# AI-ON/Few-Shot-Music-Generation

Measured on AMD Instinct MI355X. Metric: episodes/s (LSTM-baseline train step, synthetic vocab=10k seq_len=128 5-way/5-shot h=512), higher is better.
Workload: dtype f32 (bf16x3-split products, fp32 accumulate)

## Files before the change

### few-shot-music-generation_amd/csrc/api_forward.hip

```cpp
#include "fsmg_model.h"

using namespace fsmg;
using namespace fsmg_host;

namespace fsmg_host {

int stage_tokens(fsmg_model* h, const int32_t* support, int n_sup, const int32_t* query, int n_qry, int on_device) {
    const size_t T = h->T;
    if (on_device && h->eager_call) {
        h->cur_sup = support; h->cur_qry = query;
        return FSMG_OK;
    }
    const hipMemcpyKind kind = on_device ? hipMemcpyDeviceToDevice : hipMemcpyHostToDevice;
    if (n_sup > 0) HIPCK(h, hipMemcpyAsync(h->d_tok, support, sizeof(int) * n_sup * T, kind, h->stream));
    if (n_qry > 0) HIPCK(h, hipMemcpyAsync(h->d_tok + n_sup * T, query, sizeof(int) * n_qry * T, kind, h->stream));
    h->cur_sup = h->d_tok; h->cur_qry = h->d_tok + n_sup * T;
    return FSMG_OK;
}

int reset_tok_table(fsmg_model* h) {
    if (!h->tok_first) return FSMG_OK;
    OpBatch ops(h);
    GEMMCK(ops.add(h->tok_first, 0x7FFFFFFFu, h->V1));
    GEMMCK(ops.add(h->tok_count, 0u, h->V1));
    return ops.flush();
}

int token_prep(fsmg_model* h, int n_sup, int n_qry, bool train) {
    const bool table = train && h->tok_first != nullptr;
    HIPCK(h, launch_token_prep(h->stream, h->cur_sup, n_sup, h->cur_qry, n_qry, h->T, h->V, h->V,
                               h->X, h->Y, h->d_err, table ? h->tok_first : nullptr, table ? h->tok_count : nullptr));
    return FSMG_OK;
}

GemmArgs logits_args(fsmg_model* h, int B, int t0, int t1) {
    const int Hp = h->Hp;
    const int64_t r0 = (int64_t)t0 * B, m = (int64_t)(t1 - t0) * B;
    GemmArgs g{};
    g.A = h->Hs[h->L - 1] + (size_t)B * Hp + (size_t)r0 * Hp; g.lda = Hp;
    g.B = h->P + h->off_w; g.ldb = h->V1p;
    g.C = h->logits + (size_t)r0 * h->V1p; g.ldc = h->V1p; g.M = (int)m; g.N = h->V1p; g.K = Hp;
    g.bias = h->P + h->off_d; g.ksplit = 1; g.nt_store = 1;
    return g;
}
inline void fused_softmax_args(fsmg_model* h, GemmArgs& g) {
    g.ce_part = h->ce_part; g.ce_nvocab = h->V1; g.ce_store = 1;
}
int ce_finish(fsmg_model* h, hipStream_t s, int B, int64_t rows) {
    ScopedTimer tm(h, "ce");
    HIPCK(h, launch_ce_finish(s, h->ce_part, h->ce_nparts, h->Y, (int)rows, (float)(1.0 / ((double)rows + 1e-12)), h->logits, h->V1p,
                              h->lse, h->ce, h->crow, h->Hs[h->L - 1] + (size_t)B * h->Hp, h->Hsc, h->Hp, h->d_err, h->d_counters + 4));
    return FSMG_OK;
}
int ce_rows(fsmg_model* h, hipStream_t s, int B, int t0, int t1, int64_t rows_total) {
    ScopedTimer tm(h, "ce");
    const int64_t r0 = (int64_t)t0 * B, m = (int64_t)(t1 - t0) * B;
    HIPCK(h, launch_ce_rows(s, h->logits + (size_t)r0 * h->V1p, h->V1p, (int)m, h->V1, h->Y + r0, h->lse + r0,
                            h->ce + r0, dlogits_buf(h) + (size_t)r0 * h->V1p, (float)(1.0 / ((double)rows_total + 1e-12))));
    return FSMG_OK;
}

int logits_and_ce(fsmg_model* h, const Lane& ln, int B, int t0, int t1, int64_t rows_total, bool want_dlogits) {
    const int64_t r0 = (int64_t)t0 * B, m = (int64_t)(t1 - t0) * B;
    GemmArgs g = logits_args(h, B, t0, t1);
    if (!want_dlogits) {
        ScopedTimer tm(h, "gemm_logits");
        g.ce_part = h->ce_part + (size_t)r0 * h->ce_nparts; g.ce_tgt = h->Y + r0; g.ce_tgt_logit = h->tgt_logit + r0;
        g.ce_nvocab = h->V1; g.bx3 = h->bx3;
        if (use_h_gemm(h, OP_KC, OP_XC, g, ln)) g.bx3 = 3;
        else if (use_ws_gemm(h, OP_KC, OP_XC, g, ln)) { g.bx3 = 2; g.group_m = 4; }
        HIPCK(h, launch_gemm(ln.s, OP_KC, OP_XC, g, ln.lds_pad));
        HIPCK(h, launch_ce_combine(ln.s, h->ce_part + (size_t)r0 * h->ce_nparts, h->ce_nparts,
                                   h->tgt_logit + r0, (int)m, h->ce + r0));
        return FSMG_OK;
    }
// ... 219 lines not shown
```

### few-shot-music-generation_amd/csrc/api_handle.hip

```cpp
#include <mutex>
#include "fsmg_model.h"

using namespace fsmg;
using namespace fsmg_host;

namespace fsmg_host {

thread_local std::string g_create_error;

static int pick_concurrent_aux(fsmg_model* h, int priority, int max_tries) {
    if (max_tries <= 0) {
        if (hipStreamCreateWithPriority(&h->aux, hipStreamNonBlocking, priority) != hipSuccess) return fail(h, FSMG_ERR_HIP, "aux stream create failed");
        h->aux_tries = 0;
        return FSMG_OK;
    }
    int* d = nullptr;
    if (hipMalloc((void**)&d, 256) != hipSuccess) return fail(h, FSMG_ERR_NOMEM, "hipMalloc(queue probe) failed");
    auto probe = [&](hipStream_t cand, long long ticks) -> int {
        int seen = 0;
        const int init[2] = {0, -1};
        if (hipStreamSynchronize(h->stream) != hipSuccess || hipMemcpy(d, init, sizeof(init), hipMemcpyHostToDevice) != hipSuccess ||
            launch_queue_probe(h->stream, d, d + 1, 0, ticks) != hipSuccess || launch_queue_probe(cand, d, d + 1, 1, 0) != hipSuccess ||
            hipStreamSynchronize(cand) != hipSuccess || hipStreamSynchronize(h->stream) != hipSuccess ||
            hipMemcpy(&seen, d + 1, sizeof(int), hipMemcpyDeviceToHost) != hipSuccess) return -1;
// ... 100 lines not shown
        return fail(nullptr, FSMG_ERR_NO_DEVICE, std::string("libfsmg is built for gfx950 only, device is ") + prop.gcnArchName);

    fsmg_model* h = new (std::nothrow) fsmg_model();
    if (!h) return fail(nullptr, FSMG_ERR_NOMEM, "host allocation failed");
    h->cfg = *cfg;
    h->device = cfg->device;
    compute_dims(*cfg, h);
    h->n_flat = build_layout(h);
    auto bail = [&](int code, const std::string& msg) { g_create_error = msg; fsmg_destroy(h); return code; };

    if (cfg->stream) { h->stream = (hipStream_t)cfg->stream; h->own_stream = false; }
    else {
        if (hipStreamCreateWithFlags(&h->stream, hipStreamNonBlocking) != hipSuccess) return bail(FSMG_ERR_HIP, "hipStreamCreate failed");
        h->own_stream = true;
    }
    {
        if (const char* eg = std::getenv("FSMG_GRAPH")) h->cfg.use_graph = (eg[0] != '0');
        h->overlap = (int64_t)h->V1 >= 8LL * h->H * h->L;
        if (cfg->schedule == FSMG_SCHEDULE_SINGLE_STREAM) { h->overlap = false; h->overlap_forced = true; }
        if (cfg->schedule == FSMG_SCHEDULE_TWO_STREAM) { h->overlap = true; h->overlap_forced = true; }
        if (cfg->schedule == FSMG_SCHEDULE_XCD_PARTITIONED) h->xov = true;
        if (cfg->gemm == FSMG_GEMM_F32) h->bx3 = 0;
        if (cfg->recurrence == FSMG_RECURRENCE_PER_STEP) h->persist = false;
        if (cfg->recurrence == FSMG_RECURRENCE_COLUMN_SPLIT) h->xcd = false;
        if (cfg->recurrence == FSMG_RECURRENCE_XCD_LOCAL) h->pair_mode = 2;
        if (cfg->dp_split_backward) h->dp_split = cfg->dp_split_backward == 2 ? 2 : 1;
        const char* env = std::getenv("FSMG_OVERLAP");
        if (env) { h->overlap = env[0] != '0'; h->overlap_forced = true; }
        if (const char* e = std::getenv("FSMG_GEMM")) h->bx3 = std::strcmp(e, "f32") != 0;
        if (const char* e = std::getenv("FSMG_XCD_OVERLAP")) h->xov = std::atoi(e) != 0;
        if (const char* e = std::getenv("FSMG_XOV_PARTS")) h->xov_parts = std::max(1, std::min(7, std::atoi(e)));
        if (const char* e = std::getenv("FSMG_EAGER")) h->eager = (e[0] != '0');
        if (const char* e = std::getenv("FSMG_MERGE_DK")) h->merge_dk = (e[0] != '0');
        if (const char* e = std::getenv("FSMG_UPD_SPLIT")) h->upd_split = (e[0] != '0');
        if (const char* e = std::getenv("FSMG_TAIL_ASIDE")) h->tail_aside = (e[0] != '0');
        if (const char* e = std::getenv("FSMG_LAZY_CS")) h->lazy_cs = (e[0] != '0');
        if (const char* e = std::getenv("FSMG_FUSED_SOFTMAX")) h->fused_softmax = (e[0] != '0');

        if (const char* e = std::getenv("FSMG_INPLACE_DLOGITS")) h->inplace_dlogits = (e[0] != '0');
        if (const char* e = std::getenv("FSMG_XOV_SELFCHECK")) h->xov_selfcheck_left = std::max(0, std::atoi(e));
        if (const char* e = std::getenv("FSMG_XOV_SELFCHECK_EVERY")) h->xov_selfcheck_every = std::max(0, std::atoi(e));
        if (const char* e = std::getenv("FSMG_PERSISTENT")) h->persist = (e[0] != '0');
        h->persist_cfg = h->persist;
        if (const char* e = std::getenv("FSMG_FALLBACK_STEPS")) h->fallback_steps = std::max(1, std::atoi(e));
        if (const char* e = std::getenv("FSMG_XCD")) h->xcd = (e[0] != '0');
        if (const char* e = std::getenv("FSMG_XCD_PAIR")) h->pair_mode = std::max(0, std::min(2, std::atoi(e)));
        if (const char* e = std::getenv("FSMG_FWD_RT")) h->force_fwd_rt = (e[0] != '0');
        if (const char* e = std::getenv("FSMG_CHAIN_SPIN_LIMIT")) h->chain_spin_limit = std::max(0, std::atoi(e));
        if (const char* e = std::getenv("FSMG_XCD_VARIANT")) h->xcd_variant = std::atoi(e);
        if (const char* e = std::getenv("FSMG_XCD_VARIANT_BWD")) h->xcd_variant_bwd = std::atoi(e);
#ifdef FSMG_EXPERIMENTS
        if (const char* e = std::getenv("FSMG_CE_TAIL")) h->ce_tail = (e[0] != '0');
        if (const char* e = std::getenv("FSMG_CE_TAIL_BLOCKS")) h->ce_tail_blocks = std::max(1, std::min(4096, std::atoi(e)));
        if (const char* e = std::getenv("FSMG_XOV_DW_SPLIT")) h->xov_dw_split = std::max(1, std::atoi(e));
        if (const char* e = std::getenv("FSMG_XOV_PUB")) h->xov_pub = std::max(1, std::min(64, std::atoi(e)));
        if (const char* e = std::getenv("FSMG_FILL_EARLY")) h->fill_early = (e[0] != '0');
        if (const char* e = std::getenv("FSMG_FILLS_LATE")) h->fills_late = (e[0] != '0');
        if (const char* e = std::getenv("FSMG_XOV_TAIL")) h->xov_tail = std::max(0, std::min(64, std::atoi(e)));
        if (const char* e = std::getenv("FSMG_BWD_RS")) h->bwd_rs = (e[0] != '0');
        if (const char* e = std::getenv("FSMG_DP_SPLIT")) h->dp_split = std::max(0, std::min(2, std::atoi(e)));
        if (const char* e = std::getenv("FSMG_XCD_MAX_ROWS")) h->xcd_max_rows = std::max(1, std::min(128, std::atoi(e)));
        if (const char* e = std::getenv("FSMG_PERSIST_FWD")) h->persist_fwd = (e[0] != '0');
        if (const char* e = std::getenv("FSMG_PERSIST_BWD")) h->persist_bwd = (e[0] != '0');
        if (const char* e = std::getenv("FSMG_NCHUNK")) h->nchunk = h->nchunk_persist = std::max(1, std::min((int)fsmg_model::NCHUNK, std::atoi(e)));
        if (const char* e = std::getenv("FSMG_CHUNK_STEPS")) {
            std::vector<int> edges{0};
// ... 276 lines not shown
```

### few-shot-music-generation_amd/csrc/api_schedule.hip

```cpp
#include "fsmg_model.h"

using namespace fsmg;
using namespace fsmg_host;

namespace fsmg_host {

bool use_ws_gemm(fsmg_model* h, int amode, int bmode, const GemmArgs& g, const Lane& ln) {
    static const int mode = std::getenv("FSMG_GEMM_WS") ? std::atoi(std::getenv("FSMG_GEMM_WS")) : 1;
    if (!h->bx3 || mode == 0 || ln.lds_pad != 0 || g.xcd_first != 0) return false;
    if (mode == 2) return true;
    const int64_t tiles = ((g.M + 127) / 128) * (int64_t)((g.N + 127) / 128);
    if (amode == OP_KC && bmode == OP_XC) return g.K >= 384 && g.K <= 640 && tiles >= 512;
    if (amode == OP_XC && bmode == OP_XC) return tiles >= 256 && g.M <= 512;
    return g.K <= 4096;
}

bool use_h_gemm(fsmg_model* h, int amode, int bmode, const GemmArgs& g, const Lane& ln) {
    static const int mode = std::getenv("FSMG_GEMM_H") ? std::atoi(std::getenv("FSMG_GEMM_H")) : 1;
    if (!h->bx3 || mode == 0 || ln.lds_pad != 0 || g.xcd_first != 0) return false;
    if (amode == OP_XC && g.gather != nullptr && g.m_split == 0) return false;
    if (mode == 2) return true;
    const int64_t tiles = ((g.M + 255) / 256) * (int64_t)((g.N + 255) / 256);
    if (amode == OP_KC && bmode == OP_KC) return g.K >= 4096 && tiles >= 32;
    if (amode == OP_XC && bmode == OP_XC) {
        if (g.m_split > 0 && tiles >= 64) return g.K >= 896;
        return g.K >= 2048 && tiles >= 16;
    }
    return g.K >= 384 && tiles >= 512;
}

int gemm(fsmg_model* h, const Lane& ln, int amode, int bmode, GemmArgs g, OpBatch* defer, double* sq, bool* sq_done) {
    hipStream_t s = ln.s;
    g.bx3 = h->bx3;
    if (sq_done) *sq_done = false;
    int slots = ln.slots, tile_mn = 0;
    if (use_h_gemm(h, amode, bmode, g, ln)) {
        g.bx3 = 3; slots = 256; tile_mn = 256;
    } else if (use_ws_gemm(h, amode, bmode, g, ln)) {
        g.bx3 = 2; slots = 512 * 4 / 3;
        if (amode == OP_KC && bmode == OP_XC) g.group_m = 4;
    }
    const int S = (g.ldc == g.N) ? pick_split(g.M, g.N, g.K, slots, g.bx3 != 0, tile_mn) : 1;
    const int64_t mn = (int64_t)g.M * g.N;
    float* slabs = ln.slabs; float* cslabs = ln.colsum_slabs;
    bool deferred = false;
    if (S > 1 && defer != nullptr && ln.s == h->stream && h->arena != nullptr) {
        const int64_t need = round_up((int64_t)S * mn, 64) + (g.colsum ? round_up((int64_t)S * g.N, 64) : 0);
        if (h->arena_off + need <= h->arena_cap) {
            slabs = h->arena + h->arena_off; cslabs = slabs + round_up((int64_t)S * mn, 64);
            h->arena_off += need;
            deferred = true;
        }
    }
    if (S <= 1 || (!deferred && (int64_t)S * mn > h->slab_cap)) {
        if (S > 1 && !h->warned_split) {
            h->warned_split = true;
            fprintf(stderr, "[fsmg] split-K of a %d x %d x %d GEMM dropped: %d slabs do not fit the slab buffer (%lld floats)\n", g.M, g.N, g.K, S, (long long)h->slab_cap);
        }
        g.ksplit = 1;
        HIPCK(h, launch_gemm(s, amode, bmode, g, ln.lds_pad));
        if (g.row_scale != nullptr) HIPCK(h, launch_scale_rows(s, g.C, g.row_scale, g.M, g.N));
        return FSMG_OK;
    }
    if (!deferred && slabs == h->slabs && h->slabs_owner != nullptr) GEMMCK(h->slabs_owner->flush());
    if (!deferred && slabs == h->slabs && h->side_pending) {
        HIPCK(h, hipStreamWaitEvent(h->stream, h->ev_side, 0));
// ... 14 lines not shown
    }
    HIPCK(h, launch_reduce_slabs2(s, slabs, mn, S, C, mn, cslabs, g.N, colsum, colsum ? g.N : 0));
    if (g.row_scale != nullptr) HIPCK(h, launch_scale_rows(s, C, g.row_scale, g.M, g.N));
    return FSMG_OK;
}

int select_xcd_format(fsmg_model* h, int B) {
    if (h->Hp != 1024 || !h->bx3 || h->xcd_bx3_forced || h->khx == nullptr || !(h->persist && h->xcd)) return FSMG_OK;
    const bool want = lstm_xcd_bx3_pays(B, (int)h->Hp) && B <= h->xcd_max_rows;
    if (want == h->xcd_bx3) return FSMG_OK;
    h->xcd_bx3 = want;
    drop_graphs(h);
    return repack_recurrent_weights(h, h->stream);
}

void choose_schedule(fsmg_model* h, int B, bool train) {
    h->ov_call = h->overlap && (h->overlap_forced || !use_xcd(h, B));
    h->xov_call = false;
    h->eager_call = h->eager && !h->ov_call && h->persist && h->persist_fwd && h->persist_bwd &&
                    (use_xcd(h, B) || lstm_fwd_chain_supported(B, h->Hp) || lstm_fwd_chain_rt_supported(B, h->Hp));
    if (train && h->xov && ((h->Hp == 512 && h->L == 1) || h->Hp == 1024) && h->xcd_bx3 && h->bx3 && !h->ov_call && h->aux != nullptr && use_xcd(h, B) && h->persist_fwd && h->persist_bwd &&
        (!h->timing || h->timing_only == "lstm_fwd" || h->timing_only == "lstm_bwd")) {
        const int rpx = lstm_xcd16_packed_rows(B, h->Hp);
        h->xov_call = rpx > 0 && xov_first_free(B, h->Hp) <= (h->Hp == 1024 ? 6 : 5);
        if (h->xov_call) h->eager_call = true;
    }
}
void xov_gate(fsmg_model* h, GemmArgs& g, int B) {
    const int rpx = lstm_xcd16_packed_rows(B, h->Hp);
    g.gate = h->xov_prog; g.gate_expect = lstm_xcd_active_blocks(B, rpx, h->Hp); g.gate_rows = B; g.gate_last = h->T - 1;
    g.gate_err = h->d_err; g.gate_spin = h->chain_spin_limit > 0 ? 200000 : 0; g.gate_every = h->xov_pub;
}
int gemm_restricted(fsmg_model* h, hipStream_t s, int amode, int bmode, GemmArgs g, int first, int* ctl) {
    g.bx3 = 3; g.xcd_first = first; g.work = ctl; g.stop = ctl + 2; g.claim = ctl + 4; g.work_limit = gemm_items(g);
#ifdef FSMG_EXPERIMENTS
    const int dbg = xov_debug();
    if (dbg & 1) g.work_limit = 0;
    if ((dbg & 1) && (dbg & (128 | 256))) g.gate = nullptr;
    if (dbg & 16) g.dbg |= 32;
    if (dbg & 8) g.dbg |= 128;
    if (dbg & 32) g.dbg |= 64;
#endif
    HIPCK(h, launch_gemm(s, amode, bmode, g, 0));
    return FSMG_OK;
}
int gemm_prepare_queue(fsmg_model* h, GemmArgs& g, int split, OpBatch* defer, bool* ok) {
    *ok = false;
    const int S = std::max(1, std::min(std::min(split, MAX_SPLIT), g.K / 256));
    const int64_t mn = (int64_t)g.M * g.N;
    const int64_t need = round_up((int64_t)S * mn, 64) + (g.colsum ? round_up((int64_t)S * g.N, 64) : 0);
    if (S < 2 || defer == nullptr || h->arena == nullptr || g.ldc != g.N || h->arena_off + need > h->arena_cap || g.row_scale != nullptr) return FSMG_OK;
    float* slabs = h->arena + h->arena_off; float* cslabs = slabs + round_up((int64_t)S * mn, 64);
    h->arena_off += need;
    float* C = g.C; float* colsum = g.colsum;
    g.C = slabs; g.c_slab = mn; g.ksplit = S; g.bx3 = 3;
    if (colsum) { g.colsum = cslabs; g.colsum_slab = g.N; }
    if (!xov_fits(g)) { h->arena_off -= need; g.C = C; g.colsum = colsum; g.ksplit = 1; return FSMG_OK; }
    GEMMCK(defer->room(colsum ? 2 : 1));
    GEMMCK(defer->reduce(slabs, mn, S, C, mn));
    if (colsum) GEMMCK(defer->reduce(cslabs, g.N, S, colsum, g.N));
    *ok = true;
    return FSMG_OK;
}
int gemm_cleanup(fsmg_model* h, hipStream_t s, int amode, int bmode, GemmArgs g, int* ctl) {
    g.bx3 = 3; g.xcd_first = -1; g.work = ctl; g.claim = ctl + 4;
#ifdef FSMG_EXPERIMENTS
    if ((xov_debug() & 1) && (xov_debug() & (128 | 256))) g.gate = nullptr;
#endif
    HIPCK(h, launch_gemm(s, amode, bmode, g, 0));
    return FSMG_OK;
}

}
```

### few-shot-music-generation_amd/csrc/fsmg_kernels.h

```cpp
#pragma once
#include <hip/hip_runtime.h>
#include <stdint.h>

namespace fsmg {

enum { OP_KC = 0, OP_XC = 1 };
struct GemmArgs {
    const float* A; int lda;
    const float* B; int ldb;
    float* C; int ldc;
    int M, N, K;
    const float* bias;
    const int* gather;
    float* colsum;
    int ksplit;
    long long c_slab;
    long long colsum_slab;
    float2* ce_part; const int* ce_tgt; float* ce_tgt_logit; int ce_nvocab;
    int ce_store;
    const float* colsum_w;
    const float* row_scale;
    int nt_store;
    int xcd_first; int* work; int* claim; int work_limit; const int* stop;
    const int* gate; int gate_expect; int gate_rows; int gate_last; int* gate_err; int gate_spin;
    int gate_every;
    int bx3;
    int group_m;
    unsigned long long* prof;
    int dbg;
    const float* A2; int lda2; int m_split;
    int* done;
    const void* Apl; const void* Bpl;
};
inline long long plane_image_k8(int K) { return 2LL * ((K + 15) / 16); }
inline long long plane_image_bytes(int K, int X) { return 3LL * plane_image_k8(K) * X * 16; }
hipError_t launch_split_planes(hipStream_t s, int mode, const float* src, int ld, int K, int X, void* planes);
hipError_t launch_gemm(hipStream_t s, int amode, int bmode, const GemmArgs& g, int lds_pad = 0);
int gemm_lds_pad_for(int blocks_per_cu);
int gemm_block_slots();
int gemm_tile_m();
bool gemm_dma_enabled();
hipError_t launch_reduce_slabs(hipStream_t s, const float* slabs, long long slab_stride, int nslab,
                               float* out, long long n);
hipError_t launch_reduce_slabs2(hipStream_t s, const float* slabs, long long slab_stride, int nslab, float* out, long long n,
                                const float* slabs2, long long slab_stride2, float* out2, long long n2);

struct LstmFwdArgs {
    const float* KhF;
    const float* hF_prev;
    float* hF_next;
    float* z;
    const float* c_prev;
    float* c_next;
    float* h_next;
    int B, Hp;
};
hipError_t launch_lstm_fwd_step(hipStream_t s, const LstmFwdArgs& a, unsigned long long* prof = nullptr);

struct LstmFwdChainArgs {
    const float* KhF;
    float* HF;
    float* Z;
    float* Cs;
    float* Hs;
    int* err_flag;
// ... 209 lines not shown
```

### few-shot-music-generation_amd/csrc/fsmg_model.h

```cpp
#pragma once
#include <atomic>
#include <hip/hip_runtime.h>
#include <dlfcn.h>

#include <algorithm>
#include <cmath>
#include <cstdlib>
#include <new>
#include <cstdio>
#include <cstring>
#include <map>
#include <mutex>
#include <string>
#include <vector>

#include "../../include/fsmg.h"
#include "fsmg_kernels.h"

namespace fsmg_host {
using namespace fsmg;
struct OpBatch;

inline int64_t round_up(int64_t x, int64_t m) { return (x + m - 1) / m * m; }

// ... 90 lines not shown
    int ticket_next = 0;
    int64_t n_timeouts = 0, n_persist_launches = 0, n_xcd_launches = 0, n_step_launches = 0;
    bool khf_dirty = true;
    bool lazy_cs = true;
    bool cs_stale = false;
    float* slabs = nullptr;
    float* arena = nullptr;
    int64_t arena_cap = 0, arena_off = 0;
    bool warned_split = false;
    int* tok_first = nullptr; int* tok_count = nullptr;
    bool tok_table_open = false;
    bool last_bwd_xcd = false;
    bool eager = true, eager_call = false;
    const int* cur_sup = nullptr; const int* cur_qry = nullptr;
    bool fills_late = false;
    bool fill_early = false;
    float* colsum_slabs = nullptr;
    float* slabs2 = nullptr;
    float* colsum_slabs2 = nullptr;
    hipStream_t probe = nullptr;
    unsigned long long* d_probe = nullptr;
    hipStream_t aux = nullptr;
    int aux_tries = 0;
    static constexpr int NCHUNK = 16;
    std::vector<int> chunk_edges;
    int nchunk = 8;
    int nchunk_persist = 4;
    int aux_blocks_persist = 2;
    bool aux_blocks_from_env = false;
    int aux_blocks_per_cu = 2;
    hipEvent_t ev_chunk[NCHUNK] = {};
    hipEvent_t ev_fork = nullptr, ev_join = nullptr;
    bool merge_dk = true;
    hipEvent_t ev_bucket[2] = {};
    bool overlap = true;
    bool overlap_forced = false;
    bool ov_call = false;
    int bx3 = 1;
    bool xov = false, xov_call = false;
    bool xov_eligible = false;
    bool bucket0_recorded = false;
    int xov_dw_split = 4;
    int xov_tail = 0;
    int xov_pub = 6;
    int xov_strikes = 0;
    bool xov_last = false;
    int xov_parts = 3;
    int* xov_prog = nullptr;
    static constexpr int XOV_CTL = 8192;
    int* xov_ctl = nullptr;
    int64_t slab_cap = 0;
    std::map<std::string, hipGraphExec_t> graphs;
    struct LaunchCounts { int64_t xcd = 0, persist = 0, step = 0; bool bwd_xcd = false; };
    std::map<std::string, LaunchCounts> graph_counts;
    float* dec = nullptr;
    char* gen = nullptr;
    size_t gen_bytes = 0;

#ifdef FSMG_PHASE_DEBUG
    hipEvent_t ph[8] = {}; bool ph_init = false; int ph_step = 0;
#endif
    void* comm = nullptr; bool own_comm = false; int world = 1, rank = 0;
    hipStream_t comm_stream = nullptr;
    hipEvent_t ev_comm = nullptr;
    int lastB = 0;
    bool have_grads = false;
// ... 300 lines not shown
```

### few-shot-music-generation_amd/csrc/gemm.hip

```cpp
#include "fsmg_kernels.h"
#include <cstdlib>
#include <algorithm>
#include <type_traits>

namespace fsmg {

typedef float f32x16 __attribute__((ext_vector_type(16)));

namespace {

#ifndef FSMG_GEMM_BK
#define FSMG_GEMM_BK 16
#endif
#ifndef FSMG_GEMM_BM
#define FSMG_GEMM_BM 128
#endif
constexpr int BM = FSMG_GEMM_BM, BN = 128, BK = FSMG_GEMM_BK;
constexpr int NTHREADS = 2 * BM;
constexpr int NWAVES = NTHREADS / 64;
constexpr int KQ = BK / 4;
template <int XW> struct Nld { static constexpr int v = XW * BK / 4 / NTHREADS; };
template <int MODE, int XW> struct TileLd { static constexpr int v = (MODE == OP_KC) ? XW + 1 : XW + 4; };

template <int XW>
// ... 979 lines not shown
            for (int pl = 2; pl >= 0; --pl)
#pragma unroll
                for (int i = 0; i < 2; ++i) {
                    a[pl][i] = *reinterpret_cast<const bf16x8_t*>(at + pl * A_PLANE + fa + i * 512);
                    b[2 - pl][i] = *reinterpret_cast<const bf16x8_t*>(bt + (2 - pl) * BX_PLANE + fb + i * 512);
                }
#define BX_TERM(PA, PB)                                                                                        \
            acc[0][0] = __builtin_amdgcn_mfma_f32_32x32x16_bf16(a[PA][0], b[PB][0], acc[0][0], 0, 0, 0);            \
            acc[0][1] = __builtin_amdgcn_mfma_f32_32x32x16_bf16(a[PA][0], b[PB][1], acc[0][1], 0, 0, 0);            \
            acc[1][0] = __builtin_amdgcn_mfma_f32_32x32x16_bf16(a[PA][1], b[PB][0], acc[1][0], 0, 0, 0);            \
            acc[1][1] = __builtin_amdgcn_mfma_f32_32x32x16_bf16(a[PA][1], b[PB][1], acc[1][1], 0, 0, 0);
            BX_TERM(2, 0) BX_TERM(0, 2) BX_TERM(1, 1) BX_TERM(1, 0) BX_TERM(0, 1) BX_TERM(0, 0)
#undef BX_TERM
            BX_STAMP(2)
            bx_barrier();
            BX_STAMP(4)
        }
        if (PROF) p_exit_loop = __builtin_amdgcn_s_memtime();
        bx_barrier();
        store_tile(g, acc, reinterpret_cast<float*>(smem), z, m0, n0, tn, tilesN, wave, lane);
    }
    if (PROF && g.prof != nullptr && lane == 0) {
        __builtin_amdgcn_s_waitcnt(0);
        const unsigned long long p_end = __builtin_amdgcn_s_memtime();
        unsigned hw, xcc;
        asm volatile("s_getreg_b32 %0, hwreg(HW_REG_HW_ID)" : "=s"(hw));
        asm volatile("s_getreg_b32 %0, hwreg(HW_REG_XCC_ID)" : "=s"(xcc));
        unsigned long long* o = g.prof + ((size_t)(blockIdx.y * gridDim.x + blockIdx.x) * (NMW + 4) + wave) * 8;
        o[0] = p_entry; o[1] = p_loop; o[2] = pacc[2]; o[3] = pacc[3]; o[4] = pacc[4]; o[5] = p_exit_loop; o[6] = p_end;
        o[7] = ((unsigned long long)xcc << 32) | hw;
    }
}

template <int AMODE, int BMODE, bool PROF = false, int BUFM = 0, bool QUEUE = false, bool AG = false, int PLM = 0>
__global__ __launch_bounds__(512, 1) void k_gemm_bx3h(const GemmArgs g) {
    constexpr int XT = 256;
    constexpr int PLANE = 2 * XT * 16, OPER = 3 * PLANE;
    constexpr int EPI = 8 * 32 * 68 * 4;
    constexpr bool DMA = BUFM >= 3;
    constexpr bool APL = (PLM & 1) != 0, BPL = (PLM & 2) != 0;
    constexpr int NSA = APL ? 3 : 2, NSB = BPL ? 3 : 2;
    constexpr int A_BYTES = NSA * OPER, PIPE = (NSA + NSB) * OPER;
    static_assert(PIPE >= EPI, "the epilogue's transpose slices live in the pipeline's LDS");
    constexpr int RAW = DMA ? ((AMODE == OP_XC && !APL) + (BMODE == OP_XC && !BPL)) * 8 * 2048 : 0;
    __shared__ __attribute__((aligned(1024))) unsigned char smem[PIPE + RAW];
    __shared__ float s_cs[256];
    const int tid = threadIdx.x;
    const int lane = tid & 63, wave = __builtin_amdgcn_readfirstlane(tid >> 6);
    const int wm = (wave >> 2) & 1, wn = wave & 3;
    const bool late = wave >= 4;
    const int l31 = lane & 31, khalf = lane >> 5;
    const int tilesM = (g.M + XT - 1) / XT, tilesN = (g.N + XT - 1) / XT;
    int tm, tn, z;
    if (QUEUE) {
        __shared__ int s_item;
        const int total = tilesM * tilesN * (g.ksplit > 1 ? g.ksplit : 1);
        if (g.xcd_first > 0) {
            int xcc;
            asm volatile("s_getreg_b32 %0, hwreg(HW_REG_XCC_ID)" : "=s"(xcc));
            if ((xcc & 7) < g.xcd_first) {
#ifdef FSMG_EXPERIMENTS
                if (g.dbg & 64) return;
#endif
                if (g.gate == nullptr) return;
                if (tid == 0) s_item = __hip_atomic_load(g.gate + g.gate_last, __ATOMIC_RELAXED, __HIP_MEMORY_SCOPE_AGENT) >= g.gate_expect;
                __syncthreads();
                const int join = s_item;
                __syncthreads();
                if (!join) return;
            }
        }
        if (tid == 0) {
            int item = -1;
            if (g.xcd_first < 0) {
// ... 81 lines not shown
    const bool cs_weighted = WCS && do_colsum && g.colsum_w != nullptr;
    const float* cs_p = (WCS && g.colsum_w != nullptr ? g.colsum_w : g.B) + kb + 8 * ((DMA && BMODE == OP_XC) ? (lane >> 5) : (tid >> 8)) + (lane & 7);
    float cs_wv = 0.0f;
    unsigned char* const smemB = smem + A_BYTES;
    constexpr int NLD_A = APL ? 3 : (AMODE == OP_KC ? 2 : (DMA ? 2 : 8)), NLD_B = BPL ? 3 : (BMODE == OP_KC ? 2 : (DMA ? 2 : 8));
    constexpr int NLD = NLD_A + NLD_B + (WCS ? 1 : 0);
#define BXH_FETCH(T, S3)                                                                                       \
    if constexpr (APL) sa.fetch(smem + (S3) * OPER);                                                           \
    if constexpr (BPL) sb.fetch(smemB + (S3) * OPER);                                                          \
    if ((T) < nfull) { if constexpr (!APL) sa.fetch(); if constexpr (!BPL) sb.fetch(); }                       \
    else { if constexpr (!APL) sa.fetch_partial(kb + (T) * 16, ke, tid); if constexpr (!BPL) sb.fetch_partial(kb + (T) * 16, ke, tid); } \
    if constexpr (WCS) cs_wv = cs_p[(T) * 16];
#define BXH_COMMIT(ST)                                                                                         \
    if constexpr (!APL) sa.load();                                                                             \
    if constexpr (!BPL) {                                                                                      \
    sb.load();                                                                                                 \
    if (do_colsum) {                                                                                           \
        if (cs_weighted) {                \
            csum = fmaf(sb.v[0], cs_bcast<0>(cs_wv), csum); csum = fmaf(sb.v[1], cs_bcast<1>(cs_wv), csum);   \
            csum = fmaf(sb.v[2], cs_bcast<2>(cs_wv), csum); csum = fmaf(sb.v[3], cs_bcast<3>(cs_wv), csum);   \
            csum = fmaf(sb.v[4], cs_bcast<4>(cs_wv), csum); csum = fmaf(sb.v[5], cs_bcast<5>(cs_wv), csum);   \
            csum = fmaf(sb.v[6], cs_bcast<6>(cs_wv), csum); csum = fmaf(sb.v[7], cs_bcast<7>(cs_wv), csum);   \
        } else csum += sb.sum8();                                                                              \
    }                                                                                                          \
    }                                                                                                          \
    if constexpr (!APL) sa.commit(smem + (ST) * OPER);                                                         \
    if constexpr (!BPL) sb.commit(smemB + (ST) * OPER);
#define BXH_WAIT_PLANES(T1)                                                                                    \
    if constexpr (PLM != 0) {                                                                                  \
        if ((T1) + 1 < nfull) asm volatile("s_waitcnt vmcnt(%0)" :: "n"(NLD) : "memory");                      \
        else asm volatile("s_waitcnt vmcnt(0)" ::: "memory");                                                  \
    }

    if (nk > 0) {
        BXH_FETCH(0, 0)
        BXH_COMMIT(0)
        if (nk > 1) { BXH_FETCH(1, 1) }
        BXH_WAIT_PLANES(0)
    }
    bx_barrier();
    const int fa = khalf * (XT * 16) + (wm * 128 + l31) * 16, fb = khalf * (XT * 16) + (wn * 64 + l31) * 16;
    if (PROF) { p_loop = plast = __builtin_amdgcn_s_memtime(); }
    int s3 = 0;
    for (int kt = 0; kt < nk; ++kt) {
        const bool more = kt + 1 < nk;
        const int s3n = s3 == 0 ? 2 : s3 - 1;
        constexpr bool READS_ALL_FIRST = (AMODE == OP_KC && BMODE == OP_KC) || PLM != 0;
        const unsigned char* at = smem + (APL ? s3 : (kt & 1)) * OPER;
        const unsigned char* bt = smemB + (BPL ? s3 : (kt & 1)) * OPER;
        bf16x8_t a[3][4], b[3][2];
        if constexpr (PLM == 3) { if (kt + 2 < nk) { BXH_FETCH(kt + 2, s3n) } }
#define BXH_READ_A(pl) _Pragma("unroll") for (int i = 0; i < 4; ++i) a[pl][i] = *reinterpret_cast<const bf16x8_t*>(at + (pl) * PLANE + fa + i * 512);
#define BXH_READ_B(pl) _Pragma("unroll") for (int j = 0; j < 2; ++j) b[pl][j] = *reinterpret_cast<const bf16x8_t*>(bt + (pl) * PLANE + fb + j * 512);
        BXH_READ_A(2) BXH_READ_B(0)
        if (READS_ALL_FIRST) { BXH_READ_A(0) BXH_READ_B(2) BXH_READ_A(1) BXH_READ_B(1) }
        __builtin_amdgcn_sched_barrier(0);
        if constexpr (PLM != 3) if (late && more) {
            BXH_COMMIT((kt + 1) & 1)
            if (kt + 2 < nk) { BXH_FETCH(kt + 2, s3n) }
        }
        __builtin_amdgcn_sched_barrier(0);
        BX_STAMP(3)
        if (!READS_ALL_FIRST) { BXH_READ_A(0) BXH_READ_B(2) BXH_READ_A(1) BXH_READ_B(1) }
#undef BXH_READ_A
#undef BXH_READ_B
#define BXH_TERM(PA, PB)                                                                                       \
        _Pragma("unroll") for (int i = 0; i < 4; ++i)                                                          \
        _Pragma("unroll") for (int j = 0; j < 2; ++j)                                                          \
            acc[i][j] = __builtin_amdgcn_mfma_f32_32x32x16_bf16(a[PA][i], b[PB][j], acc[i][j], 0, 0, 0);
        BXH_TERM(2, 0) BXH_TERM(0, 2) BXH_TERM(1, 1) BXH_TERM(1, 0) BXH_TERM(0, 1) BXH_TERM(0, 0)
#undef BXH_TERM
        BX_STAMP(2)
        if constexpr (PLM != 3) if (!late && more) {
            BXH_COMMIT((kt + 1) & 1)
            if (kt + 2 < nk) { BXH_FETCH(kt + 2, s3n) }
        }
        BX_STAMP(3)
        if (more) { BXH_WAIT_PLANES(kt + 1) }
        bx_barrier();
        BX_STAMP(4)
        s3 = s3 == 2 ? 0 : s3 + 1;
    }
#undef BXH_FETCH
#undef BXH_COMMIT
#undef BXH_WAIT_PLANES
    const unsigned long long p_exit_loop = PROF ? __builtin_amdgcn_s_memtime() : 0;

    if (do_colsum) {
        const int col = (DMA && BMODE == OP_XC) ? 32 * wave + (lane & 31) : (tid & 255);
        const bool upper = (DMA && BMODE == OP_XC) ? lane >= 32 : tid >= 256;
        if (upper) s_cs[col] = csum;
        bx_barrier();
        if (!upper && n0 + col < g.N) g.colsum[(long long)z * g.colsum_slab + n0 + col] = csum + s_cs[col];
    }
    float* ep = reinterpret_cast<float*>(smem) + wave * (32 * 68);
    if (PROF && (g.dbg & 8)) {
        float sink = 0.0f;
#pragma unroll
        for (int i = 0; i < 4; ++i)
#pragma unroll
            for (int j = 0; j < 2; ++j)
#pragma unroll
                for (int r = 0; r < 16; ++r) sink += acc[i][j][r];
        if (sink == 1.2345e-30f) g.C[0] = sink;
    } else
#pragma unroll
    for (int h2 = 0; h2 < 2; ++h2) {
        if ((n0 + wn * 64) / 128 >= (g.N + 127) / 128) break;
        f32x16 (&sub)[2][2] = *reinterpret_cast<f32x16 (*)[2][2]>(&acc[2 * h2][0]);
        store_tile_at(g, sub, ep, z, m0 + wm * 128 + h2 * 64, n0 + wn * 64, (n0 + wn * 64) / 128, (g.N + 127) / 128, wn & 1, lane);
    }
#ifdef FSMG_EXPERIMENTS
    if constexpr (QUEUE) {
        if (g.done != nullptr) {
// ... 40 lines not shown
            return hipErrorInvalidValue;
        }
        dim3 grid3(((g.M + 255) / 256) * ((g.N + 255) / 256), g.ksplit > 1 ? g.ksplit : 1);
        if (plm == 3) { hipLaunchKernelGGL((k_gemm_bx3h<AMODE, BMODE, false, 2, false, false, 3>), grid3, dim3(512), lds_pad, s, g); return hipGetLastError(); }
        if constexpr (AMODE == OP_KC) {
            if (plm == 2) { hipLaunchKernelGGL((k_gemm_bx3h<AMODE, BMODE, false, 2, false, false, 2>), grid3, dim3(512), lds_pad, s, g); return hipGetLastError(); }
        }
        if constexpr (BMODE == OP_KC) {
            if (plm == 1) { hipLaunchKernelGGL((k_gemm_bx3h<AMODE, BMODE, false, 2, false, false, 1>), grid3, dim3(512), lds_pad, s, g); return hipGetLastError(); }
        }
        return hipErrorInvalidValue;
#endif
    }
    if (g.xcd_first != 0 && g.bx3 == 3) {
        if (g.work == nullptr || g.claim == nullptr || (g.xcd_first > 0 && g.stop == nullptr) || g.gather != nullptr || g.prof != nullptr) return hipErrorInvalidValue;
        const long long a_b = 4LL * g.lda * (AMODE == OP_KC ? g.M : g.K), b_b = 4LL * g.ldb * (BMODE == OP_KC ? g.N : g.K);
        if (a_b >= 0xfffff000LL || b_b >= 0xfffff000LL) return hipErrorInvalidValue;
        const int total = ((g.M + 255) / 256) * ((g.N + 255) / 256) * (g.ksplit > 1 ? g.ksplit : 1);
        const int lim = g.work_limit < total ? g.work_limit : total;
        const int blocks = g.xcd_first > 0 ? (int)(((long long)lim * 8 + 7 - g.xcd_first) / (8 - g.xcd_first)) + 64 : total;
        const bool a_dma = AMODE != OP_XC || (g.lda % 4 == 0 && g.M % 4 == 0 && ((uintptr_t)g.A & 15) == 0);
        const bool b_dma = BMODE != OP_XC || (g.ldb % 4 == 0 && g.N % 4 == 0 && ((uintptr_t)g.B & 15) == 0);
        if constexpr (AMODE == OP_XC && BMODE == OP_XC) {
            if (g.m_split > 0) {
                const bool ok = g.m_split % 256 == 0 && g.m_split < g.M && g.A2 != nullptr && b_dma && g.lda % 4 == 0 && g.lda2 % 4 == 0 &&
                                (g.M - g.m_split) % 4 == 0 && (((uintptr_t)g.A | (uintptr_t)g.A2) & 15) == 0 && 4LL * g.lda2 * g.K < 0xfffff000LL;
                if (!ok) return hipErrorInvalidValue;
                hipLaunchKernelGGL((k_gemm_bx3h<AMODE, BMODE, false, 3, true, true>), dim3(blocks), dim3(512), 0, s, g);
                return hipGetLastError();
            }
            if (a_dma && b_dma) { hipLaunchKernelGGL((k_gemm_bx3h<AMODE, BMODE, false, 3, true>), dim3(blocks), dim3(512), 0, s, g); return hipGetLastError(); }
        }
        if (g.m_split > 0) return hipErrorInvalidValue;
        hipLaunchKernelGGL((k_gemm_bx3h<AMODE, BMODE, false, 2, true>), dim3(blocks), dim3(512), 0, s, g);
        return hipGetLastError();
    }
    if (g.xcd_first != 0) {
        if (g.work == nullptr || g.claim == nullptr || (g.xcd_first > 0 && g.stop == nullptr) || (AMODE == OP_XC && g.gather != nullptr)) return hipErrorInvalidValue;
        const int total = tilesM * tilesN * (g.ksplit > 1 ? g.ksplit : 1);
        const int lim = g.work_limit < total ? g.work_limit : total;
        const int blocks = g.xcd_first > 0 ? (int)(((long long)lim * 8 + 7 - g.xcd_first) / (8 - g.xcd_first)) + 64 : total;
        hipLaunchKernelGGL((k_gemm_queue<AMODE, BMODE>), dim3(blocks), dim3(NTHREADS), lds_pad, s, g);
        return hipGetLastError();
    }
    dim3 grid(tilesM * tilesN, g.ksplit > 1 ? g.ksplit : 1);
    const long long a_bytes = 4LL * g.lda * (AMODE == OP_KC ? g.M : g.K), b_bytes = 4LL * g.ldb * (BMODE == OP_KC ? g.N : g.K);
    const bool a_buf = g.gather == nullptr && a_bytes < 0xfffff000LL, b_buf = b_bytes < 0xfffff000LL;
    static const bool buf_off = std::getenv("FSMG_GEMM_BUF") && std::atoi(std::getenv("FSMG_GEMM_BUF")) == 0;
    const int bufm = (buf_off && g.prof == nullptr) ? 0 : (a_buf && b_buf) ? 2 : (b_buf ? 1 : 0);
#ifdef FSMG_EXPERIMENTS
    if (g.prof != nullptr && bufm != 2) return hipErrorInvalidValue;
#else
    if (g.prof != nullptr) return hipErrorInvalidValue;
#endif
    if (g.bx3 == 3) {
        dim3 grid3(((g.M + 255) / 256) * ((g.N + 255) / 256), g.ksplit > 1 ? g.ksplit : 1);
        if (g.m_split > 0) {
            if constexpr (AMODE == OP_XC && BMODE == OP_XC) {
                const bool ok = g.m_split % 256 == 0 && g.m_split < g.M && g.A2 != nullptr && g.prof == nullptr && b_buf &&
                                g.lda % 4 == 0 && g.lda2 % 4 == 0 && (g.M - g.m_split) % 4 == 0 && g.ldb % 4 == 0 && g.N % 4 == 0 &&
                                (((uintptr_t)g.A | (uintptr_t)g.A2 | (uintptr_t)g.B) & 15) == 0 && 4LL * g.lda2 * g.K < 0xfffff000LL &&
                                (g.gather != nullptr || 4LL * g.lda * g.K < 0xfffff000LL);
                if (!ok) return hipErrorInvalidValue;
                hipLaunchKernelGGL((k_gemm_bx3h<AMODE, BMODE, false, 3, false, true>), grid3, dim3(512), lds_pad, s, g);
                return hipGetLastError();
            }
            return hipErrorInvalidValue;
        }
        const bool dma_off = !gemm_dma_enabled();
        const bool a_dma = AMODE != OP_XC || (g.lda % 4 == 0 && g.M % 4 == 0 && ((uintptr_t)g.A & 15) == 0);
        const bool b_dma = BMODE != OP_XC || (g.ldb % 4 == 0 && g.N % 4 == 0 && ((uintptr_t)g.B & 15) == 0);
        const bool dma = !dma_off && bufm == 2 && a_dma && b_dma;
        if constexpr (AMODE == OP_XC && BMODE == OP_XC) {
#ifdef FSMG_EXPERIMENTS
            if (dma && g.prof != nullptr) { hipLaunchKernelGGL((k_gemm_bx3h<AMODE, BMODE, true, 3>), grid3, dim3(512), lds_pad, s, g); return hipGetLastError(); }
#endif
            if (dma) { hipLaunchKernelGGL((k_gemm_bx3h<AMODE, BMODE, false, 3>), grid3, dim3(512), lds_pad, s, g); return hipGetLastError(); }
        }
#ifdef FSMG_EXPERIMENTS
        if (g.prof != nullptr) { hipLaunchKernelGGL((k_gemm_bx3h<AMODE, BMODE, true, 2>), grid3, dim3(512), lds_pad, s, g); return hipGetLastError(); }
#endif
        if (bufm == 2) hipLaunchKernelGGL((k_gemm_bx3h<AMODE, BMODE, false, 2>), grid3, dim3(512), lds_pad, s, g);
        else if (bufm == 1) hipLaunchKernelGGL((k_gemm_bx3h<AMODE, BMODE, false, 1>), grid3, dim3(512), lds_pad, s, g);
        else hipLaunchKernelGGL((k_gemm_bx3h<AMODE, BMODE>), grid3, dim3(512), lds_pad, s, g);
        return hipGetLastError();
    }
    if (g.bx3 == 2) {
#ifdef FSMG_EXPERIMENTS
        if (g.prof != nullptr) { hipLaunchKernelGGL((k_gemm_bx3w<AMODE, BMODE, 1, true, 2>), grid, dim3(512), lds_pad, s, g); return hipGetLastError(); }
#endif
        if (bufm == 2) hipLaunchKernelGGL((k_gemm_bx3w<AMODE, BMODE, 1, false, 2>), grid, dim3(512), lds_pad, s, g);
        else if (bufm == 1) hipLaunchKernelGGL((k_gemm_bx3w<AMODE, BMODE, 1, false, 1>), grid, dim3(512), lds_pad, s, g);
        else hipLaunchKernelGGL((k_gemm_bx3w<AMODE, BMODE, 1>), grid, dim3(512), lds_pad, s, g);
        return hipGetLastError();
    }
    if (g.bx3) {
#ifdef FSMG_EXPERIMENTS
        if (g.prof != nullptr) { hipLaunchKernelGGL((k_gemm_bx3<AMODE, BMODE, true, 2>), grid, dim3(256), lds_pad, s, g); return hipGetLastError(); }
#endif
        if (bufm == 2) hipLaunchKernelGGL((k_gemm_bx3<AMODE, BMODE, false, 2>), grid, dim3(256), lds_pad, s, g);
        else if (bufm == 1) hipLaunchKernelGGL((k_gemm_bx3<AMODE, BMODE, false, 1>), grid, dim3(256), lds_pad, s, g);
        else hipLaunchKernelGGL((k_gemm_bx3<AMODE, BMODE>), grid, dim3(256), lds_pad, s, g);
        return hipGetLastError();
    }
    if (AMODE == OP_XC && g.gather != nullptr) hipLaunchKernelGGL((k_gemm_staged<OP_XC, OP_XC>), grid, dim3(NTHREADS), lds_pad, s, g);
    else hipLaunchKernelGGL((k_gemm<AMODE, BMODE>), grid, dim3(NTHREADS), lds_pad, s, g);
    return hipGetLastError();
}

template <int MODE>
__global__ __launch_bounds__(256) void k_split_planes(const float* __restrict__ src, int ld, int K, int X, uint4* __restrict__ planes) {
// ... 104 lines not shown
```

Baseline: 618.7.

## Add triple-buffered software-pipelined K loop to bx3 GEMM for KC x XC operands

Adds a P3 variant of the bf16x3 high-tile GEMM kernel that uses three LDS stages for both operands. It prefetches the next stage's first fragments into registers before the barrier so the LDS reads for the next k-tile overlap the current MFMA work. The variant is selected by default for OP_KC x OP_XC GEMMs, both queue-based and grid launches, when register-staged buffering applies, and can be turned off with FSMG_GEMM_PIPE=0. In exchange it uses more LDS and more live registers, which could lower occupancy or cause spills.

```diff
diff --git a/few-shot-music-generation_amd/csrc/api_forward.hip b/few-shot-music-generation_amd/csrc/api_forward.hip
--- a/few-shot-music-generation_amd/csrc/api_forward.hip
+++ b/few-shot-music-generation_amd/csrc/api_forward.hip
@@ -40,7 +40,7 @@
     g.A = h->Hs[h->L - 1] + (size_t)B * Hp + (size_t)r0 * Hp; g.lda = Hp;
     g.B = h->P + h->off_w; g.ldb = h->V1p;
     g.C = h->logits + (size_t)r0 * h->V1p; g.ldc = h->V1p; g.M = (int)m; g.N = h->V1p; g.K = Hp;
-    g.bias = h->P + h->off_d; g.ksplit = 1; g.nt_store = 1;
+    g.bias = h->P + h->off_d; g.ksplit = 1; g.nt_store = 1; g.pipe_off = !h->gemm_pipe;
     return g;
 }
 inline void fused_softmax_args(fsmg_model* h, GemmArgs& g) {
diff --git a/few-shot-music-generation_amd/csrc/api_handle.hip b/few-shot-music-generation_amd/csrc/api_handle.hip
--- a/few-shot-music-generation_amd/csrc/api_handle.hip
+++ b/few-shot-music-generation_amd/csrc/api_handle.hip
@@ -156,6 +156,7 @@
         if (const char* e = std::getenv("FSMG_XOV_PARTS")) h->xov_parts = std::max(1, std::min(7, std::atoi(e)));
         if (const char* e = std::getenv("FSMG_EAGER")) h->eager = (e[0] != '0');
         if (const char* e = std::getenv("FSMG_MERGE_DK")) h->merge_dk = (e[0] != '0');
+        if (const char* e = std::getenv("FSMG_GEMM_PIPE")) h->gemm_pipe = (e[0] != '0');
         if (const char* e = std::getenv("FSMG_UPD_SPLIT")) h->upd_split = (e[0] != '0');
         if (const char* e = std::getenv("FSMG_TAIL_ASIDE")) h->tail_aside = (e[0] != '0');
         if (const char* e = std::getenv("FSMG_LAZY_CS")) h->lazy_cs = (e[0] != '0');
diff --git a/few-shot-music-generation_amd/csrc/api_schedule.hip b/few-shot-music-generation_amd/csrc/api_schedule.hip
--- a/few-shot-music-generation_amd/csrc/api_schedule.hip
+++ b/few-shot-music-generation_amd/csrc/api_schedule.hip
@@ -31,7 +31,7 @@
 
 int gemm(fsmg_model* h, const Lane& ln, int amode, int bmode, GemmArgs g, OpBatch* defer, double* sq, bool* sq_done) {
     hipStream_t s = ln.s;
-    g.bx3 = h->bx3;
+    g.bx3 = h->bx3; g.pipe_off = !h->gemm_pipe;
     if (sq_done) *sq_done = false;
     int slots = ln.slots, tile_mn = 0;
     if (use_h_gemm(h, amode, bmode, g, ln)) {
@@ -112,7 +112,7 @@
     g.gate_err = h->d_err; g.gate_spin = h->chain_spin_limit > 0 ? 200000 : 0; g.gate_every = h->xov_pub;
 }
 int gemm_restricted(fsmg_model* h, hipStream_t s, int amode, int bmode, GemmArgs g, int first, int* ctl) {
-    g.bx3 = 3; g.xcd_first = first; g.work = ctl; g.stop = ctl + 2; g.claim = ctl + 4; g.work_limit = gemm_items(g);
+    g.bx3 = 3; g.xcd_first = first; g.work = ctl; g.stop = ctl + 2; g.claim = ctl + 4; g.work_limit = gemm_items(g); g.pipe_off = !h->gemm_pipe;
 #ifdef FSMG_EXPERIMENTS
     const int dbg = xov_debug();
     if (dbg & 1) g.work_limit = 0;
@@ -143,7 +143,7 @@
     return FSMG_OK;
 }
 int gemm_cleanup(fsmg_model* h, hipStream_t s, int amode, int bmode, GemmArgs g, int* ctl) {
-    g.bx3 = 3; g.xcd_first = -1; g.work = ctl; g.claim = ctl + 4;
+    g.bx3 = 3; g.xcd_first = -1; g.work = ctl; g.claim = ctl + 4; g.pipe_off = !h->gemm_pipe;
 #ifdef FSMG_EXPERIMENTS
     if ((xov_debug() & 1) && (xov_debug() & (128 | 256))) g.gate = nullptr;
 #endif
diff --git a/few-shot-music-generation_amd/csrc/fsmg_kernels.h b/few-shot-music-generation_amd/csrc/fsmg_kernels.h
--- a/few-shot-music-generation_amd/csrc/fsmg_kernels.h
+++ b/few-shot-music-generation_amd/csrc/fsmg_kernels.h
@@ -31,6 +31,7 @@
     const float* A2; int lda2; int m_split;
     int* done;
     const void* Apl; const void* Bpl;
+    int pipe_off;
 };
 inline long long plane_image_k8(int K) { return 2LL * ((K + 15) / 16); }
 inline long long plane_image_bytes(int K, int X) { return 3LL * plane_image_k8(K) * X * 16; }
diff --git a/few-shot-music-generation_amd/csrc/fsmg_model.h b/few-shot-music-generation_amd/csrc/fsmg_model.h
--- a/few-shot-music-generation_amd/csrc/fsmg_model.h
+++ b/few-shot-music-generation_amd/csrc/fsmg_model.h
@@ -146,6 +146,7 @@
     hipEvent_t ev_chunk[NCHUNK] = {};
     hipEvent_t ev_fork = nullptr, ev_join = nullptr;
     bool merge_dk = true;
+    bool gemm_pipe = true;
     hipEvent_t ev_bucket[2] = {};
     bool overlap = true;
     bool overlap_forced = false;
diff --git a/few-shot-music-generation_amd/csrc/gemm.hip b/few-shot-music-generation_amd/csrc/gemm.hip
--- a/few-shot-music-generation_amd/csrc/gemm.hip
+++ b/few-shot-music-generation_amd/csrc/gemm.hip
@@ -1035,14 +1035,15 @@
     }
 }
 
-template <int AMODE, int BMODE, bool PROF = false, int BUFM = 0, bool QUEUE = false, bool AG = false, int PLM = 0>
+template <int AMODE, int BMODE, bool PROF = false, int BUFM = 0, bool QUEUE = false, bool AG = false, int PLM = 0, bool P3 = false>
 __global__ __launch_bounds__(512, 1) void k_gemm_bx3h(const GemmArgs g) {
     constexpr int XT = 256;
     constexpr int PLANE = 2 * XT * 16, OPER = 3 * PLANE;
     constexpr int EPI = 8 * 32 * 68 * 4;
     constexpr bool DMA = BUFM >= 3;
     constexpr bool APL = (PLM & 1) != 0, BPL = (PLM & 2) != 0;
-    constexpr int NSA = APL ? 3 : 2, NSB = BPL ? 3 : 2;
+    static_assert(!P3 || (PLM == 0 && !DMA && !AG), "pipelined loop: register-staged operands only (3 x 32 KiB LDS-DMA regions do not fit)");
+    constexpr int NSA = (APL || P3) ? 3 : 2, NSB = (BPL || P3) ? 3 : 2;
     constexpr int A_BYTES = NSA * OPER, PIPE = (NSA + NSB) * OPER;
     static_assert(PIPE >= EPI, "the epilogue's transpose slices live in the pipeline's LDS");
     constexpr int RAW = DMA ? ((AMODE == OP_XC && !APL) + (BMODE == OP_XC && !BPL)) * 8 * 2048 : 0;
@@ -1190,6 +1191,67 @@
         else asm volatile("s_waitcnt vmcnt(0)" ::: "memory");                                                  \
     }
 
+    if constexpr (P3) {
+    const int fa = khalf * (XT * 16) + (wm * 128 + l31) * 16, fb = khalf * (XT * 16) + (wn * 64 + l31) * 16;
+    if (nk > 0) {
+        BXH_FETCH(0, 0)
+        BXH_COMMIT(0)
+        if (nk > 1) { BXH_FETCH(1, 0) BXH_COMMIT(1) }
+        if (nk > 2) { BXH_FETCH(2, 0) }
+    }
+    bx_barrier();
+    bf16x8_t a2n[4], b0n[2];
+#define BXH_READ_FIRST(ST)                                                                                     \
+    _Pragma("unroll") for (int i = 0; i < 4; ++i) a2n[i] = *reinterpret_cast<const bf16x8_t*>(smem + (ST) * OPER + 2 * PLANE + fa + i * 512); \
+    _Pragma("unroll") for (int j = 0; j < 2; ++j) b0n[j] = *reinterpret_cast<const bf16x8_t*>(smemB + (ST) * OPER + fb + j * 512);
+    if (nk > 0) { BXH_READ_FIRST(0) }
+    if (PROF) { p_loop = plast = __builtin_amdgcn_s_memtime(); }
+    int s3 = 0;
+    for (int kt = 0; kt < nk; ++kt) {
+        const int s3n = s3 == 2 ? 0 : s3 + 1, s3w = s3 == 0 ? 2 : s3 - 1;
+        const bool commit = kt + 2 < nk;
+        const unsigned char* at = smem + s3 * OPER;
+        const unsigned char* bt = smemB + s3 * OPER;
+        bf16x8_t a[3][4], b[3][2];
+#pragma unroll
+        for (int i = 0; i < 4; ++i) a[2][i] = a2n[i];
+#pragma unroll
+        for (int j = 0; j < 2; ++j) b[0][j] = b0n[j];
+        if (late && commit) {
+            BXH_COMMIT(s3w)
+            if (kt + 3 < nk) { BXH_FETCH(kt + 3, 0) }
+        }
+        __builtin_amdgcn_sched_barrier(0);
+        BX_STAMP(3)
+#pragma unroll
+        for (int i = 0; i < 4; ++i) a[0][i] = *reinterpret_cast<const bf16x8_t*>(at + fa + i * 512);
+#pragma unroll
+        for (int j = 0; j < 2; ++j) b[2][j] = *reinterpret_cast<const bf16x8_t*>(bt + 2 * PLANE + fb + j * 512);
+#pragma unroll
+        for (int i = 0; i < 4; ++i) a[1][i] = *reinterpret_cast<const bf16x8_t*>(at + PLANE + fa + i * 512);
+#pragma unroll
+        for (int j = 0; j < 2; ++j) b[1][j] = *reinterpret_cast<const bf16x8_t*>(bt + PLANE + fb + j * 512);
+#define BXH_TERM(PA, PB)                                                                                       \
+        _Pragma("unroll") for (int i = 0; i < 4; ++i)                                                          \
+        _Pragma("unroll") for (int j = 0; j < 2; ++j)                                                          \
+            acc[i][j] = __builtin_amdgcn_mfma_f32_32x32x16_bf16(a[PA][i], b[PB][j], acc[i][j], 0, 0, 0);
+        BXH_TERM(2, 0) BXH_TERM(0, 2) BXH_TERM(1, 1) BXH_TERM(1, 0) BXH_TERM(0, 1) BXH_TERM(0, 0)
+#undef BXH_TERM
+        __builtin_amdgcn_sched_barrier(0);
+        BX_STAMP(2)
+        if (!late && commit) {
+            BXH_COMMIT(s3w)
+            if (kt + 3 < nk) { BXH_FETCH(kt + 3, 0) }
+        }
+        __builtin_amdgcn_sched_barrier(0);
+        if (kt + 1 < nk) { BXH_READ_FIRST(s3n) }
+        BX_STAMP(3)
+        bx_barrier();
+        BX_STAMP(4)
+        s3 = s3n;
+    }
+#undef BXH_READ_FIRST
+    } else {
     if (nk > 0) {
         BXH_FETCH(0, 0)
         BXH_COMMIT(0)
@@ -1238,6 +1300,7 @@
         bx_barrier();
         BX_STAMP(4)
         s3 = s3 == 2 ? 0 : s3 + 1;
+    }
     }
 #undef BXH_FETCH
 #undef BXH_COMMIT
@@ -1344,6 +1407,9 @@
             if (a_dma && b_dma) { hipLaunchKernelGGL((k_gemm_bx3h<AMODE, BMODE, false, 3, true>), dim3(blocks), dim3(512), 0, s, g); return hipGetLastError(); }
         }
         if (g.m_split > 0) return hipErrorInvalidValue;
+        if constexpr (AMODE == OP_KC && BMODE == OP_XC) {
+            if (!g.pipe_off) { hipLaunchKernelGGL((k_gemm_bx3h<AMODE, BMODE, false, 2, true, false, 0, true>), dim3(blocks), dim3(512), 0, s, g); return hipGetLastError(); }
+        }
         hipLaunchKernelGGL((k_gemm_bx3h<AMODE, BMODE, false, 2, true>), dim3(blocks), dim3(512), 0, s, g);
         return hipGetLastError();
     }
@@ -1389,6 +1455,15 @@
 #endif
             if (dma) { hipLaunchKernelGGL((k_gemm_bx3h<AMODE, BMODE, false, 3>), grid3, dim3(512), lds_pad, s, g); return hipGetLastError(); }
         }
+        if constexpr (AMODE == OP_KC && BMODE == OP_XC) {
+            if (!g.pipe_off && bufm == 2 && lds_pad == 0) {
+#ifdef FSMG_EXPERIMENTS
+                if (g.prof != nullptr) { hipLaunchKernelGGL((k_gemm_bx3h<AMODE, BMODE, true, 2, false, false, 0, true>), grid3, dim3(512), 0, s, g); return hipGetLastError(); }
+#endif
+                hipLaunchKernelGGL((k_gemm_bx3h<AMODE, BMODE, false, 2, false, false, 0, true>), grid3, dim3(512), 0, s, g);
+                return hipGetLastError();
+            }
+        }
 #ifdef FSMG_EXPERIMENTS
         if (g.prof != nullptr) { hipLaunchKernelGGL((k_gemm_bx3h<AMODE, BMODE, true, 2>), grid3, dim3(512), lds_pad, s, g); return hipGetLastError(); }
 #endif
```

After: 621.8 (median of 6 runs). Within noise of the previous version (+0.5%).
